# roxas1533/pathtrace

Measured on AMD Instinct MI355X. Metric: Msamples/sec (pixels x spp / s) at 1024^2/64spp, higher is better.
Workload: dtype f32; 1 GPU; C2: 10-sphere diffuse Cornell scene, 1024x1024, 64 spp, MIS, min_depth 4 / max_depth 50; hit_scene=linear scan (reference), launch=one process, one GPU, tiles=whole image

## Files before the change

include/pathtrace_amd.h:

```cpp
#ifndef PATHTRACE_AMD_H
#define PATHTRACE_AMD_H

#include <stdint.h>

#ifdef __cplusplus
extern "C" {
#endif

#define PT_ABI_VERSION 6

typedef enum {
    PT_OK = 0,
    PT_ERR_INVALID_ARG = 1,
    PT_ERR_NO_DEVICE = 2,
    PT_ERR_HIP = 3,
    PT_ERR_OOM = 4,
    PT_ERR_UNSUPPORTED = 5
} PtStatus;


typedef struct {
    double origin[3];
    double lower_left[3];
    double horizontal[3];
// ... 204 lines not shown
                                float* out_noisy_linear, float* out_features);

int pt_ray_color(PtContext* ctx, const PtRenderParams* params, const double* rays,
                 const uint32_t* xy, uint32_t n, float* out_rgb);

int pt_debug_hit_scene(PtContext* ctx, const double* rays, uint32_t n,
                       double t_min, double t_max, uint32_t exact_math, uint32_t accel,
                       int32_t* out_id, float* out_t);

int pt_debug_hit_records(PtContext* ctx, const double* rays, uint32_t n,
                         double t_min, double t_max, uint32_t exact_math, uint32_t accel,
                         int32_t* out_id, float* out_rec);

int pt_debug_bsdf_eval(PtContext* ctx, uint32_t obj, const double* in10, uint32_t n, uint32_t exact_math, float* out4);
int pt_debug_bsdf_sample(PtContext* ctx, uint32_t obj, const double* in7, const uint32_t* words4, uint32_t n,
                         uint32_t exact_math, float* out8);
int pt_debug_shape_sample(PtContext* ctx, uint32_t obj, const double* from3, const double* target3, const double* r12,
                          uint32_t n, uint32_t exact_math, float* out8);
int pt_debug_light_point(PtContext* ctx, const double* from3, const uint32_t* words4, uint32_t n, uint32_t exact_math,
                         float* out8);
int pt_debug_camera_rays(PtContext* ctx, const PtCamera* cam, const uint32_t* xys, uint32_t n, uint32_t exact_math,
                         float* out8);

int pt_debug_bvh_check(const PtObject* objs, uint32_t n_objs, uint32_t* depth, uint32_t* n_nodes,
                       uint32_t* n_leaf_slots);

const char* pt_last_error(void);
uint32_t pt_abi_version(void);

#ifdef __cplusplus
}
#endif
#endif
```

pathtrace_amd/_lib.py:

```python
import ctypes as C
import os

_HERE = os.path.dirname(os.path.abspath(__file__))
LIB_PATH = os.environ.get("PATHTRACE_AMD_LIB") or os.path.join(_HERE, "libpathtrace_amd.so")


class PtCamera(C.Structure):
    _fields_ = [
        ("origin", C.c_double * 3),
        ("lower_left", C.c_double * 3),
        ("horizontal", C.c_double * 3),
        ("vertical", C.c_double * 3),
        ("width", C.c_uint32),
        ("height", C.c_uint32),
    ]


class PtObject(C.Structure):
    _fields_ = [
        ("shape_tag", C.c_uint32),
        ("mat_tag", C.c_uint32),
        ("shape", C.c_double * 9),
        ("mat", C.c_double * 6),
    ]
# ... 120 lines not shown
    "pt_context_set_tuning": (C.c_int, [C.c_void_p, _P(PtTuning)]),
    "pt_scene_upload": (C.c_int, [C.c_void_p, _P(PtObject), C.c_uint32]),
    "pt_render_device": (C.c_int, [C.c_void_p, _P(PtCamera), _P(PtRenderParams), C.c_void_p, C.c_void_p]),
    "pt_render_device_packed": (C.c_int, [C.c_void_p, _P(PtCamera), _P(PtRenderParams), C.c_void_p]),
    "pt_sync": (C.c_int, [C.c_void_p]),
    "pt_get_stats": (C.c_int, [C.c_void_p, _P(PtStats)]),
    "pt_debug_raw_stats": (C.c_int, [C.c_void_p, _P(C.c_uint64)]),
    "pt_debug_scan_layout": (C.c_int, [C.c_void_p, _P(C.c_uint32), _P(C.c_uint32), _P(C.c_uint32)]),
    "pt_render_host": (C.c_int, [C.c_void_p, _P(PtCamera), _P(PtRenderParams), C.c_void_p, C.c_void_p]),
    "pt_render_progressive": (C.c_int, [C.c_void_p, _P(PtCamera), _P(PtRenderParams), C.c_uint32, C.c_void_p,
                                        C.c_void_p, C.c_void_p, C.c_void_p]),
    "pt_render": (C.c_int, [_P(PtCamera), _P(PtObject), C.c_uint32, _P(PtRenderParams), C.c_void_p, C.c_void_p]),
    "pt_debug_hit_scene": (C.c_int, [C.c_void_p, _P(C.c_double), C.c_uint32, C.c_double, C.c_double, C.c_uint32,
                                     C.c_uint32, _P(C.c_int32), _P(C.c_float)]),
    "pt_debug_hit_records": (C.c_int, [C.c_void_p, _P(C.c_double), C.c_uint32, C.c_double, C.c_double, C.c_uint32,
                                       C.c_uint32, _P(C.c_int32), _P(C.c_float)]),
    "pt_debug_bsdf_eval": (C.c_int, [C.c_void_p, C.c_uint32, _P(C.c_double), C.c_uint32, C.c_uint32, _P(C.c_float)]),
    "pt_debug_bsdf_sample": (C.c_int, [C.c_void_p, C.c_uint32, _P(C.c_double), _P(C.c_uint32), C.c_uint32, C.c_uint32,
                                       _P(C.c_float)]),
    "pt_debug_shape_sample": (C.c_int, [C.c_void_p, C.c_uint32, _P(C.c_double), _P(C.c_double), _P(C.c_double), C.c_uint32,
                                        C.c_uint32, _P(C.c_float)]),
    "pt_debug_light_point": (C.c_int, [C.c_void_p, _P(C.c_double), _P(C.c_uint32), C.c_uint32, C.c_uint32, _P(C.c_float)]),
    "pt_debug_camera_rays": (C.c_int, [C.c_void_p, _P(PtCamera), _P(C.c_uint32), C.c_uint32, C.c_uint32, _P(C.c_float)]),
    "pt_debug_bvh_check": (C.c_int, [_P(PtObject), C.c_uint32, _P(C.c_uint32), _P(C.c_uint32), _P(C.c_uint32)]),
    "pt_render_pixels": (C.c_int, [C.c_void_p, _P(PtCamera), _P(PtRenderParams), _P(C.c_uint32), C.c_uint32, C.c_void_p,
                                   C.c_void_p, C.c_void_p]),
    "pt_render_adaptive": (C.c_int, [C.c_void_p, _P(PtCamera), _P(PtRenderParams), _P(PtAdaptive), C.c_void_p, C.c_void_p,
                                     C.c_void_p, C.c_void_p]),
    "pt_render_features_device": (C.c_int, [C.c_void_p, _P(PtCamera), _P(PtRenderParams), C.c_uint32, C.c_void_p]),
    "pt_default_denoise": (None, [_P(PtDenoise)]),
    "pt_denoise_device": (C.c_int, [C.c_void_p, C.c_uint32, C.c_uint32, C.c_void_p, C.c_void_p, _P(PtDenoise), C.c_void_p, C.c_void_p]),
    "pt_render_denoised": (C.c_int, [C.c_void_p, _P(PtCamera), _P(PtRenderParams), C.c_uint32, _P(PtDenoise), C.c_void_p, C.c_void_p,
                                     C.c_void_p, C.c_void_p]),
    "pt_default_temporal": (None, [_P(PtTemporal)]),
    "pt_temporal_reset": (C.c_int, [C.c_void_p]),
    "pt_denoise_temporal_device": (C.c_int, [C.c_void_p, _P(PtCamera), C.c_void_p, C.c_void_p, _P(PtDenoise), _P(PtTemporal), C.c_void_p,
                                             C.c_void_p]),
    "pt_render_denoised_temporal": (C.c_int, [C.c_void_p, _P(PtCamera), _P(PtRenderParams), C.c_uint32, _P(PtDenoise), _P(PtTemporal),
                                              C.c_void_p, C.c_void_p, C.c_void_p, C.c_void_p]),
    "pt_ray_color": (C.c_int, [C.c_void_p, _P(PtRenderParams), _P(C.c_double), _P(C.c_uint32), C.c_uint32, C.c_void_p]),
    "pt_shutdown": (None, []),
    "pt_multi_create": (C.c_int, [_P(C.c_int), C.c_uint32, _P(C.c_void_p)]),
    "pt_multi_destroy": (C.c_int, [C.c_void_p]),
    "pt_multi_device_count": (C.c_uint32, [C.c_void_p]),
    "pt_multi_set_threads": (C.c_int, [C.c_void_p, C.c_int]),
    "pt_multi_set_exchange": (C.c_int, [C.c_void_p, C.c_uint32]),
# ... 60 lines not shown
```

pathtrace_amd/csrc/pt_api.cpp:

```cpp
#include <algorithm>
#include <cmath>
#include <cstdarg>
#include <cstdio>
#include <cstdlib>
#include <cstring>
#include <mutex>
#include <string>
#include <vector>

#include "../../include/pathtrace_amd.h"
#include "pt_bvh.h"
#include "pt_kernels.h"
#include "pt_sched.h"

#ifdef PT_SAN_NO_KERNELS
namespace ptk {
uint32_t launch_path_kernel_exact(const BounceArgs&, uint32_t, hipStream_t) { std::abort(); }
uint32_t launch_path_kernel_fast(const BounceArgs&, uint32_t, hipStream_t) { std::abort(); }
void launch_resolve_adaptive(const AdaptiveResolveArgs&, hipStream_t) { std::abort(); }
void launch_adaptive_select(const uint2*, uint32_t, uint32_t, const uint32_t*, uint32_t*, uint2*, uint32_t*, hipStream_t) { std::abort(); }
void launch_feature_rays_exact(const CameraF&, uint32_t, uint32_t, float*, hipStream_t) { std::abort(); }
void launch_feature_rays_fast(const CameraF&, uint32_t, uint32_t, float*, hipStream_t) { std::abort(); }
void launch_feature_resolve_exact(const FeatureResolveArgs&, hipStream_t) { std::abort(); }
void launch_feature_resolve_fast(const FeatureResolveArgs&, hipStream_t) { std::abort(); }
// ... 1166 lines not shown
                          uint32_t n, uint32_t exact_math, float* out8) {
    if ((!from3 || (!target3 && !r12)) && n) return fail(PT_ERR_INVALID_ARG, "null argument");
    std::vector<float> in(9 * (size_t)n, 0.0f);
    for (size_t i = 0; i < n; ++i) {
        for (int k = 0; k < 3; ++k) in[9 * i + k] = (float)from3[3 * i + k];
        if (target3) { for (int k = 0; k < 3; ++k) in[9 * i + 3 + k] = (float)target3[3 * i + k]; in[9 * i + 8] = 1.0f; }
        else { in[9 * i + 6] = (float)r12[2 * i]; in[9 * i + 7] = (float)r12[2 * i + 1]; }
    }
    return debug_fn(c, ptk::kFnShapeSample, obj, in, 9, nullptr, n, 8, exact_math, nullptr, out8);
}
int pt_debug_light_point(PtContext* c, const double* from3, const uint32_t* words4, uint32_t n, uint32_t exact_math,
                         float* out8) {
    if ((!from3 || !words4) && n) return fail(PT_ERR_INVALID_ARG, "null argument");
    return debug_fn(c, ptk::kFnLightPoint, 0, to_f32(from3, 3 * (size_t)n), 3, words4, n, 8, exact_math, nullptr, out8);
}
int pt_debug_camera_rays(PtContext* c, const PtCamera* cam, const uint32_t* xys, uint32_t n, uint32_t exact_math, float* out8) {
    if ((!cam || !xys) && n) return fail(PT_ERR_INVALID_ARG, "null argument");
    if (cam && (cam->width < 2 || cam->height < 2)) return fail(PT_ERR_INVALID_ARG, "camera %ux%u: width and height must be >= 2", cam->width, cam->height);
    std::vector<uint32_t> w(4 * (size_t)n, 0u);
    for (size_t i = 0; i < n; ++i) { w[4 * i] = xys[3 * i]; w[4 * i + 1] = xys[3 * i + 1]; w[4 * i + 2] = xys[3 * i + 2]; }
    return debug_fn(c, ptk::kFnCameraRay, 0, std::vector<float>(), 1, w.data(), n, 8, exact_math, cam, out8);
}

int pt_debug_bvh_check(const PtObject* objs, uint32_t n, uint32_t* depth, uint32_t* n_nodes, uint32_t* n_leaf_slots) {
    if (!objs && n) return fail(PT_ERR_INVALID_ARG, "pt_debug_bvh_check: null objects");
    if (n >= (1u << 28)) return fail(PT_ERR_UNSUPPORTED, "accel: %u objects exceed the 2^28 leaf slots", n);
    std::vector<float4> shape(3 * (size_t)n + 1), scan(3 * (size_t)n + 1);
    std::vector<uint32_t> tag(n + 1);
    for (uint32_t i = 0; i < n; ++i) {
        if (objs[i].shape_tag > PT_SHAPE_TRIANGLE) return fail(PT_ERR_INVALID_ARG, "object %u: bad shape_tag %u", i, objs[i].shape_tag);
        int ns = 0;
        shape_records(objs[i], &shape[3 * (size_t)i], &scan[3 * (size_t)i], &ns);
        tag[i] = objs[i].shape_tag;
    }
    const ptbvh::Built b = ptbvh::build(shape.data(), tag.data(), n);
    if (depth) *depth = b.depth;
    if (n_nodes) *n_nodes = (uint32_t)b.wide.size();
    if (n_leaf_slots) *n_leaf_slots = b.leaf_prims;
    if (b.non_finite) return fail(PT_ERR_UNSUPPORTED, "accel: %u object(s) with a NaN/inf coordinate", b.non_finite);
    if (b.depth + 2u > ptbvh::kStackDepth || b.stack_need > ptbvh::kStackDepth)
        return fail(PT_ERR_UNSUPPORTED, "BVH (depth %u, stack need %u) exceeds the traversal stack", b.depth, b.stack_need);
    if (b.leaf_prims != n || b.leaf_rec.size() != 3 * b.leaf_ids.size() || b.leaf_lead.size() != b.leaf_ids.size() || b.leaf_ids.size() % 4u != 0u)
        return fail(PT_ERR_UNSUPPORTED, "%u primitives in %zu leaf slots for %u objects", b.leaf_prims, b.leaf_ids.size(), n);
    if (n == 0) return b.root == ptbvh::kDone ? PT_OK : fail(PT_ERR_UNSUPPORTED, "empty scene: root is not the sentinel");
    auto prim_box = [&](uint32_t o, double lo[3], double hi[3]) {
        const float4 r0 = shape[3 * (size_t)o], r1 = shape[3 * (size_t)o + 1], r2 = shape[3 * (size_t)o + 2];
// ... 521 lines not shown
```

pathtrace_amd/csrc/pt_kernels.h:

```cpp
#pragma once
#include <hip/hip_runtime.h>
#include <stdint.h>

namespace ptk {

enum { kRunSphere = 0, kRunTriangle = 1, kRunTrianglePair = 2 };
struct Run {
    uint32_t tag;
    uint32_t first_obj;
    uint32_t count;
    uint32_t off4;
};
constexpr uint32_t run_entry_f4(uint32_t tag) { return tag == kRunSphere ? 1u : tag == kRunTriangle ? 3u : 5u; }

struct BvhView {
    const uint4* nodes;
    float grid_min[3], grid_cell[3];
    const float4* rec;
    const float4* lead;
    const uint32_t* ids;
    uint32_t root;
    float scene_abs;
};

// ... 139 lines not shown
    AdaptiveFilm f;
    const Rgb* lsamp;
    const uint2* pixels;
    uint32_t width, n, nb, n_total;
    uint32_t load;
    uint32_t finalize;
    uint32_t* zero_words;
    uint32_t n_zero;
};
void launch_resolve_adaptive(const AdaptiveResolveArgs& a, hipStream_t st);
constexpr uint32_t kSelectTile = 1024;
void launch_adaptive_select(const uint2* pixels, uint32_t n, uint32_t width, const uint32_t* conv, uint32_t* block_counts,
                            uint2* out, uint32_t* out_n, hipStream_t st);

void launch_film_pack(const float* lin, const uint8_t* rgba, uint32_t np, void* packed, hipStream_t st);
void launch_film_unpack(const void* recv, uint32_t W, uint32_t H, uint32_t band_rows, uint32_t n_dev, uint32_t max_rows, float* lin,
                        uint8_t* rgba, hipStream_t st);

void launch_debug_hit_exact(const SceneView& sc, uint32_t accel, const float* rays6, uint32_t n, float t_min, float t_max,
                            float4* scratch, int32_t* out_id, float* out_t, float* out_rec, hipStream_t st);
void launch_debug_hit_fast(const SceneView& sc, uint32_t accel, const float* rays6, uint32_t n, float t_min, float t_max,
                           float4* scratch, int32_t* out_id, float* out_t, float* out_rec, hipStream_t st);

enum { kFnBsdfEval = 0, kFnBsdfSample = 1, kFnShapeSample = 2, kFnLightPoint = 3, kFnCameraRay = 4 };
struct DebugFnArgs {
    SceneView sc;
    CameraF cam;
    uint32_t op, obj, n;
    uint32_t in_stride, out_stride;
    const float* in;
    const uint32_t* words;
    float* out;
};
void launch_debug_fn_exact(const DebugFnArgs& a, hipStream_t st);
void launch_debug_fn_fast(const DebugFnArgs& a, hipStream_t st);


struct FeatureResolveArgs {
    const float4* mat;
    const int32_t* ids;
    const float* rec;
    float4* out;
    uint32_t np, nb, n_samples, load, finalize;
};
void launch_feature_rays_exact(const CameraF& cam, uint32_t s_base, uint32_t nb, float* rays6, hipStream_t st);
void launch_feature_rays_fast(const CameraF& cam, uint32_t s_base, uint32_t nb, float* rays6, hipStream_t st);
void launch_feature_resolve_exact(const FeatureResolveArgs& a, hipStream_t st);
// ... 26 lines not shown
```

pathtrace_amd/csrc/pt_kernels.hip:

```cpp
#include "pt_device.h"
#include "pt_kernels.h"
#include "pt_adaptive.h"

using namespace PTD_NS;
using namespace ptk;

#if PT_MATH_EXACT
#define PTK_IMPL ptk_exact_impl
#define PT_LAUNCH(name) name##_exact
#else
#define PTK_IMPL ptk_fast_impl
#define PT_LAUNCH(name) name##_fast
#endif

#ifndef PT_TU
#define PT_TU 0
#endif
#define PT_TU_MAIN (PT_TU == 0 || PT_TU == 1)
#define PT_TU_SPLIT (PT_TU == 0 || PT_TU == 2)
#define PT_TU_BVH (PT_TU == 0 || PT_TU == 3)
namespace PTK_IMPL {

template <bool ORDERED = false, bool ANY = false>
PT_DEV void sphere_test(float4 s, f3 o, f3 d, float t_min, float& closest, int& id, int obj) {
// ... 190 lines not shown
    for (uint32_t r = 0; r < sc.n_runs; ++r) {
        Run run = sc.runs[r];
        run.tag = __builtin_amdgcn_readfirstlane(run.tag); run.first_obj = __builtin_amdgcn_readfirstlane(run.first_obj);
        run.count = __builtin_amdgcn_readfirstlane(run.count); run.off4 = __builtin_amdgcn_readfirstlane(run.off4);
        const uint32_t per = run_entry_f4(run.tag);
        if (SMALL) {
            scan_run<false, ANY, PF>(sc.scan + run.off4, run.tag, run.count, (int)run.first_obj, o, d, t_min, closest, id);
        } else {
            float4* tile = const_cast<float4*>(sc.scan);
            const uint32_t tile_prims = kTileF4 / per;
            for (uint32_t p0 = 0; p0 < run.count; p0 += tile_prims) {
                uint32_t np = run.count - p0 < tile_prims ? run.count - p0 : tile_prims;
                __syncthreads();
                const float4* src = sc.scan_global + run.off4 + p0 * per;
                for (uint32_t k = threadIdx.x; k < np * per; k += kBlock) tile[k] = src[k];
                __syncthreads();
                scan_run<true, ANY>(tile, run.tag, np, (int)(run.first_obj + p0 * (run.tag == kRunTrianglePair ? 2u : 1u)), o, d, t_min, closest, id);
            }
        }
    }
    id_out = id;
    t_out = closest;
}
PT_DEV void scan_global(const SceneRef& sc, f3 o, f3 d, float t_min, float t_max, int& id_out, float& t_out) {
    float closest = t_max;
    int id = -1;
    for (uint32_t r = 0; r < sc.n_runs; ++r) {
        const Run run = sc.runs_global[r];
        scan_run<false>(sc.scan_global + run.off4, run.tag, run.count, (int)run.first_obj, o, d, t_min, closest, id);
    }
    id_out = id;
    t_out = closest;
}

PT_DEV f3 parked_origin() { return mk(3e18f, 3e18f, 3e18f); }
PT_DEV f3 parked_dir() { return mk(1.0f, 0.0f, 0.0f); }

PT_DEV uint32_t lane_rank(unsigned long long mask) {
    return __builtin_amdgcn_mbcnt_hi((uint32_t)(mask >> 32), __builtin_amdgcn_mbcnt_lo((uint32_t)mask, 0u));
}
PT_DEV void divmod_magic(uint32_t n, uint32_t d, uint32_t magic, uint32_t& q, uint32_t& r) {
    q = __umulhi(n, magic);
    r = n - q * d;
    if (r >= d) { q += 1u; r -= d; }
}
PT_DEV uint32_t image_row(const TileMap& t, uint32_t yl) {
// ... 136 lines not shown
    v.light_dir = mk(0.f, 0.f, 0.f); v.ls_emission = mk(0.f, 0.f, 0.f);
    v.distance = 0.0f; v.ls_pdf = 1.0f;
    v.w_bsdf1 = v.w_bsdf2 = v.w_lobe = v.w_rr = 0u;
    if (v.alive) {
        uint32_t ds[4];
        philox4x32_draw(kx, py, sample, p.depth, BLK_SURFACE, 0u, ds);
        v.w_bsdf1 = ds[2]; v.w_bsdf2 = ds[3];
        v.w_rr = (ds[0] << 23) | ((ds[1] & 0x1FFu) << 14) | ((ds[2] & 0x1FFu) << 5);
        if (MIS && sc.n_lights > 0u) {
            uint32_t w_index = 0u;
            if (sc.n_lights > 1u) {
                uint32_t dc[4];
                philox4x32_draw(kx, py, sample, p.depth, BLK_CHOICE, 0u, dc);
                w_index = dc[0]; v.w_lobe = dc[1];
            }
            f3 lp;
            sample_light_point<DIFFUSE>(sc, v.hit.point, w_index, ds[0], ds[1], lp, v.light_obj, v.ls_emission, v.ls_pdf,
                                        v.light_dir, v.distance);
            v.need_shadow = true;
        }
    }
}

template <bool MIS, int DIFFUSE, bool REMAT>
PT_DEV bool vertex_end(const SceneRef& sc, PathState& p, const Vertex& vin, bool visible, uint32_t sample, uint32_t kx,
                       uint32_t py, uint32_t min_depth, uint32_t max_depth) {
    const uint32_t n_lights = sc.n_lights;
    Vertex v = vin;
    if (REMAT) {
        asm volatile("" ::: "memory");
        v.m = load_mat(sc.mat, vin.obj);
        v.ls_emission = load_mat(sc.mat, vin.light_obj).color;
    }
    if (DIFFUSE != kMatsMirror) assume_mats<DIFFUSE>(v.m.tag);
    else if (vin.alive) assume_mats<DIFFUSE>(v.m.tag);
    if (vin.hit_emitter) {
        if (!MIS || p.depth == 0u) {
            p.L = p.L + p.beta * v.m.color;
        } else {
            float w_bsdf = pt_div(p.pdf_prev, p.pdf_prev + vin.emit_pdf_shape);
            p.L = p.L + p.beta * v.m.color * w_bsdf;
        }
    }
    f3 direct = mk(0.f, 0.f, 0.f);
    if (MIS && visible) {
        float cos_theta = __builtin_fabsf(dot(v.hit.normal, v.light_dir));
        f3 bsdf; float pdf_bsdf;
        bsdf_pdf(v.m, p.d, p.eta_in, v.light_dir, v.hit.normal, bsdf, pdf_bsdf);
        float w_nee = pt_div(v.ls_pdf, v.ls_pdf + pdf_bsdf);
        direct = w_nee * bsdf * v.ls_emission * cos_theta / v.ls_pdf;
    }

    bool alive = v.alive;
    if (alive) {
        uint32_t w_lobe = v.w_lobe, w_rr = v.w_rr;
        if (!(MIS && n_lights > 1u) && v.m.tag == MAT_MIRROR) {
            uint32_t dc[4];
            philox4x32_draw(kx, py, sample, p.depth, BLK_CHOICE, 0u, dc);
            w_lobe = dc[1];
        }
        float eta_mat = v.m.tag == MAT_MIRROR ? v.m.ior : 1.0f;
        float eta_here = v.hit.front_face ? pt_rcp(eta_mat) : eta_mat;
        f3 wo, bsdf; float pdf, cos_theta;
        bsdf_pdf_sample(v.m, p.d, eta_here, v.hit.normal, v.w_bsdf1, v.w_bsdf2, w_lobe, wo, bsdf, pdf, cos_theta);
        f3 next_tp = p.beta * bsdf * cos_theta / pdf;
        float rr = rr_prob(p.depth, min_depth, max_depth, next_tp);
        if (u01(w_rr) > rr) {
            alive = false;
        } else {
            p.L = p.L + p.beta * direct;
            p.beta = rr == 1.0f ? next_tp : next_tp / rr;
            if (is_zero(p.beta) || p.depth >= 65534u) {
                alive = false;
            } else {
                p.pdf_prev = pdf;
                p.o = v.hit.point;
                p.d = v.m.tag == MAT_EMISSIVE ? normalize(wo) : wo;
                p.eta_in = eta_here;
                p.depth += 1u;
            }
        }
    }
    return alive;
}

#ifndef PT_BOUNCE_WAVES_LDS
#define PT_BOUNCE_WAVES_LDS 6
#endif
#ifndef PT_BOUNCE_WAVES_TILED
#define PT_BOUNCE_WAVES_TILED 5
#endif
template <bool LIST>
PT_DEV void pixel_key(const BounceArgs& a, const PathState& p, bool active, uint32_t& kx, uint32_t& py) {
    if (LIST) { const uint2 k = a.pixels[active ? ((p.yl << 16) | p.px) : 0u]; kx = k.x; py = k.y; }
    else { kx = p.px; py = image_row(a.tile, p.yl); }
}
// ... 144 lines not shown
        const uint32_t base = s_iters[0];
        if (threadIdx.x < n_in) {
#pragma unroll 1
            for (int k = 0; k < 4; ++k) { const float4 t = a.q.q[k][seg_base + threadIdx.x]; a.ovf_out.q[k][base + threadIdx.x] = t; }
        }
    }
    if (lane == 0u) wave_totals<MIS, !OVF>(s_totals, kBlock / 64, a.stats, wave_shadow, wave_vertices, wave_samples, wave_depth);
}

constexpr uint32_t kPool = 128;
#ifndef PT_REGEN_BLOCK
#define PT_REGEN_BLOCK 256
#endif
constexpr uint32_t kRegenBlock = PT_REGEN_BLOCK;
#ifndef PT_RESOLVE_UNROLL
#define PT_RESOLVE_UNROLL 4
#endif
template <bool MIS, int DIFFUSE, bool LIST = false>
__global__ void __launch_bounds__(kRegenBlock, DIFFUSE == kMatsDiffuse ? kRegenWavesDiffuse : kRegenWavesGeneric) k_paths_regen(BounceArgs a) {
    extern __shared__ float4 lds[];
    __shared__ float4 s_pool_d[kRegenBlock / 64][kPool];
    __shared__ uint32_t s_pool_s[kRegenBlock / 64][kPool];
    __shared__ WgTotals s_totals;
    if (threadIdx.x == 0u) wg_totals_init(s_totals);
    if (a.posted != nullptr && blockIdx.x >= a.core_blocks) {
        __shared__ uint32_t s_posted;
        if (threadIdx.x == 0u) s_posted = __hip_atomic_load(a.posted, __ATOMIC_RELAXED, __HIP_MEMORY_SCOPE_SYSTEM);
        __syncthreads();
        if (s_posted - a.seq >= 2u) return;
    }
    const SceneRef sc = stage_scene<kModeLds>(a.sc, lds);
    const uint32_t lane = threadIdx.x & 63u;
    const uint32_t wib = threadIdx.x >> 6;
    float4* const pool_d = s_pool_d[wib];
    uint32_t* const pool_s = s_pool_s[wib];
    const uint32_t n_first = a.n_first;
    const uint32_t n_chunks = (n_first + 63u) >> 6;
    const uint32_t W = a.film_w;
    const f3 cam_o = mk(a.cam.origin[0], a.cam.origin[1], a.cam.origin[2]);

    const uint32_t wave = blockIdx.x * (kRegenBlock / 64) + wib, nw = gridDim.x * (kRegenBlock / 64);
    uint32_t st_next = wave;
    uint32_t ctr = blockIdx.x % kRegenCounters, ctr_dry = 0;
    uint32_t pool_head = 0, pool_cnt = 0;
    bool exhausted = false;
    uint32_t wave_shadow = 0, wave_vertices = 0;
    uint32_t wave_taken = 0;
    uint32_t dmax = 0;
    PathState p = parked_state();
    bool alive = false;
#ifdef PT_DRAIN_TIMING
    const unsigned long long t_begin = wall_clock64();
    unsigned long long t_exhausted = 0ull;
#endif

    for (;;) {
#ifdef PT_DRAIN_TIMING
        if (exhausted && t_exhausted == 0ull) t_exhausted = wall_clock64();
#endif
        while (!exhausted && pool_cnt < 64u) {
            uint32_t chunk;
            if (st_next < a.regen_static) {
                chunk = st_next; st_next += nw;
            } else {
                for (;;) {
                    uint32_t got = 0;
                    if (lane == 0u) got = atomicAdd(a.chunk_counter + ctr * kRegenCounterStride, 1u);
                    chunk = a.regen_static + __builtin_amdgcn_readfirstlane(got) * kRegenCounters + ctr;
                    if (chunk < n_chunks) break;
                    ctr = ctr + 1u == kRegenCounters ? 0u : ctr + 1u;
                    if (++ctr_dry == kRegenCounters) { exhausted = true; break; }
                }
                if (exhausted) break;
            }
            const uint32_t pid = chunk * 64u + lane;
            const uint32_t valid = n_first - chunk * 64u < 64u ? n_first - chunk * 64u : 64u;
            if (lane < valid) {
                uint32_t s_local, pix, yl, px;
                divmod_magic(pid, a.np, a.np_magic, s_local, pix);
                divmod_magic(pix, W, a.film_w_magic, yl, px);
                f3 o, d;
                if constexpr (LIST) { const uint2 k = a.pixels[pix]; camera_ray(a.cam, a.s_base + s_local, k.x, k.y, o, d); }
                else camera_ray(a.cam, a.s_base + s_local, px, image_row(a.tile, yl), o, d);
                const uint32_t e = (pool_head + pool_cnt + lane) & (kPool - 1u);
                pool_d[e] = make_float4(d.x, d.y, d.z, __uint_as_float((yl << 16) | px));
                pool_s[e] = s_local << 16;
            }
            pool_cnt += valid;
        }
        __builtin_amdgcn_wave_barrier();
        {
            const unsigned long long need = __ballot(!alive);
            const uint32_t r = lane_rank(need);
            if (!alive && r < pool_cnt) {
                const uint32_t e = (pool_head + r) & (kPool - 1u);
                const float4 q = pool_d[e];
                const uint32_t sd = pool_s[e];
                p.o = cam_o; p.d = mk(q.x, q.y, q.z);
                const uint32_t xy = __float_as_uint(q.w);
                p.yl = xy >> 16; p.px = xy & 0xFFFFu;
                p.s_local = sd >> 16; p.depth = 0u;
                p.beta = mk(1.f, 1.f, 1.f); p.L = mk(0.f, 0.f, 0.f);
                p.pdf_prev = 0.0f; p.eta_in = 1.0f;
                alive = true;
            }
            const uint32_t n_need = (uint32_t)__popcll(need);
            const uint32_t n_take = n_need < pool_cnt ? n_need : pool_cnt;
            pool_head += n_take; pool_cnt -= n_take;
            wave_taken += n_take;
        }
        __builtin_amdgcn_wave_barrier();
        const uint32_t n_alive = (uint32_t)__popcll(__ballot(alive));
        if (n_alive < a.export_below) break;

        const bool active = alive;
        uint32_t kx = p.px, py = image_row(a.tile, p.yl);
        if constexpr (LIST) pixel_key<true>(a, p, active, kx, py);
        const uint32_t sample = a.s_base + p.s_local;
        wave_vertices += n_alive;

        int id; float t;
        scan_closest<kModeLds, false>(sc, p.o, p.d, a.t_min, kInf, id, t);
        Vertex v;
        vertex_begin<MIS, DIFFUSE>(sc, p, active, id, t, sample, kx, py, v);

        bool visible = false;
        if (MIS) {
            const unsigned long long sm = __ballot(v.need_shadow);
            if (sm != 0ull) {
                f3 sdir = v.need_shadow ? v.light_dir : parked_dir();
                f3 sorg = v.need_shadow ? v.hit.point : parked_origin();
                int sid; float st;
                scan_closest<kModeLds, true>(sc, sorg, sdir, a.t_min, v.distance - a.t_min, sid, st);
                visible = v.need_shadow && sid < 0;
                wave_shadow += (uint32_t)__popcll(sm);
            }
        }
        alive = vertex_end<MIS, DIFFUSE, true>(sc, p, v, visible, sample, kx, py, a.min_depth, a.max_depth);
        if (active && !alive) {
            a.lsamp[p.s_local * a.np + p.yl * W + p.px] = Rgb{p.L.x, p.L.y, p.L.z};
            dmax = p.depth > dmax ? p.depth : dmax;
            p.o = parked_origin(); p.d = parked_dir();
        }
    }

    {
        const unsigned long long mask = __ballot(alive);
        const uint32_t n_left = (uint32_t)__popcll(mask);
        if (n_left != 0u) {
            uint32_t base = 0;
            if (lane == 0u) base = atomicAdd(a.ovf_out_count, n_left);
            base = __builtin_amdgcn_readfirstlane(base);
            if (alive) {
                store_state(a.ovf_out, base + lane_rank(mask), p);
                const uint32_t done = p.depth ? p.depth - 1u : 0u;
                dmax = done > dmax ? done : dmax;
            }
        }
        wave_taken -= n_left;
    }
    const uint32_t wave_samples = wave_taken;
    for (int off = 32; off > 0; off >>= 1) { const uint32_t w2 = (uint32_t)__shfl_xor((int)dmax, off); dmax = w2 > dmax ? w2 : dmax; }
    if (lane == 0u) {
        wave_totals<MIS>(s_totals, kRegenBlock / 64, a.stats, wave_shadow, wave_vertices, wave_samples, dmax);
#ifdef PT_DRAIN_TIMING
// ... 915 lines not shown
        const bool with_target = in[8] != 0.0f;
        shape_sample(sc.shape, sc.mat, (int)a.obj, m.shape_tag, from, with_target, mk(in[3], in[4], in[5]), in[6], in[7], point, pdf, dir, dist);
        if (with_target) {
            const f3 to_light = point - from;
            dir = normalize(to_light); dist = length(to_light);
        }
        out[0] = point.x; out[1] = point.y; out[2] = point.z; out[3] = pdf;
        out[4] = dir.x; out[5] = dir.y; out[6] = dir.z; out[7] = dist;
    } else if (a.op == kFnLightPoint) {
        f3 point = mk(0.f, 0.f, 0.f), le = point, ld = point; float pdf = 0.0f, ll = 0.0f; int lobj = -1;
        if (sc.n_lights > 0u) sample_light_point<false>(sc, mk(in[0], in[1], in[2]), w[0], w[1], w[2], point, lobj, le, pdf, ld, ll);
        out[0] = point.x; out[1] = point.y; out[2] = point.z; out[3] = le.x; out[4] = le.y; out[5] = le.z;
        out[6] = pdf; out[7] = (float)lobj;
    } else if (a.op == kFnCameraRay) {
        f3 o, d;
        camera_ray(a.cam, w[2], w[0], w[1], o, d);
        uint32_t dc[4];
        philox4x32_draw(w[0], w[1], w[2], kDepthCamera, BLK_SURFACE, 0u, dc);
        out[0] = o.x; out[1] = o.y; out[2] = o.z; out[3] = d.x; out[4] = d.y; out[5] = d.z;
        out[6] = u01(dc[0]); out[7] = u01(dc[1]);
    }
}

__global__ void k_scene_setup(float4* shape, float4* mat, uint32_t n) {
    const uint32_t i = blockIdx.x * blockDim.x + threadIdx.x;
    if (i >= n) return;
    const uint32_t bits = __float_as_uint(mat[2 * i].x);
    if (((bits >> 8) & 0xFFu) != SHAPE_TRIANGLE) return;
    float4 r0 = shape[3 * i], r1 = shape[3 * i + 1], r2 = shape[3 * i + 2];
    f3 normal; float pdf_area;
    triangle_constants(mk(r1.x, r1.y, r1.z), mk(r2.x, r2.y, r2.z), normal, pdf_area);
    r0.w = normal.x; r1.w = normal.y; r2.w = normal.z;
    shape[3 * i] = r0; shape[3 * i + 1] = r1; shape[3 * i + 2] = r2;
    mat[2 * i + 1].w = pdf_area;
}
#endif
}
namespace ptk {
using namespace PTK_IMPL;
#if PT_TU_BVH
void PT_LAUNCH(launch_debug_hit_bvh)(const SceneView& sc, uint32_t grid, size_t lds, const float* rays6, uint32_t n, float t_min, float t_max,
                                     float4* scratch, int32_t* out_id, float* out_t, float* out_rec, hipStream_t st) {
    hipLaunchKernelGGL(k_debug_hit_bvh, dim3(grid), dim3(kBlock), lds, st, sc, rays6, n, t_min, t_max, scratch,
                       scratch + n, scratch + 2 * (size_t)n, out_id, out_t, out_rec);
}
#endif
#if PT_TU_MAIN
void PT_LAUNCH(launch_scene_setup)(float4* shape, float4* mat, uint32_t n, hipStream_t st) {
    if (n == 0u) return;
    hipLaunchKernelGGL(k_scene_setup, dim3((n + kBlock - 1) / kBlock), dim3(kBlock), 0, st, shape, mat, n);
}
void PT_LAUNCH(launch_debug_fn)(const DebugFnArgs& a, hipStream_t st) {
    if (a.n == 0u) return;
    hipLaunchKernelGGL(k_debug_fn, dim3((a.n + kBlock - 1) / kBlock), dim3(kBlock), 0, st, a);
}
void PT_LAUNCH(launch_debug_hit)(const SceneView& sc, uint32_t accel, const float* rays6, uint32_t n, float t_min,
                                 float t_max, float4* scratch, int32_t* out_id, float* out_t, float* out_rec, hipStream_t st) {
    const int mode = scene_mode(sc, accel);
    const size_t lds = scene_lds_bytes(sc, mode);
    uint32_t grid = (n + kBlock - 1) / kBlock;
    if (grid > 2048u) grid = 2048u;
    if (grid == 0u) grid = 1u;
    if (mode == kModeLds)
        hipLaunchKernelGGL(k_debug_hit<kModeLds>, dim3(grid), dim3(kBlock), lds, st, sc, rays6, n, t_min, t_max, out_id, out_t, out_rec);
    else if (mode == kModeTiled)
        hipLaunchKernelGGL(k_debug_hit<kModeTiled>, dim3(grid), dim3(kBlock), lds, st, sc, rays6, n, t_min, t_max, out_id, out_t, out_rec);
    else
        PT_LAUNCH(launch_debug_hit_bvh)(sc, grid, lds, rays6, n, t_min, t_max, scratch, out_id, out_t, out_rec, st);
}
#endif

}

#if PT_TU_MAIN
namespace PTK_IMPL {
__global__ void __launch_bounds__(kBlock) k_feature_rays(CameraF cam, uint32_t s_base, uint32_t nb, float* __restrict__ rays6) {
// ... 269 lines not shown
```

rust/pathtrace-amd-sys/src/lib.rs:

```rust
#![allow(non_camel_case_types)]
use std::os::raw::{c_char, c_int, c_void};

pub const PT_ABI_VERSION: u32 = 6;

pub const PT_OK: c_int = 0;
pub const PT_ERR_INVALID_ARG: c_int = 1;
pub const PT_ERR_NO_DEVICE: c_int = 2;
pub const PT_ERR_HIP: c_int = 3;
pub const PT_ERR_OOM: c_int = 4;
pub const PT_ERR_UNSUPPORTED: c_int = 5;

pub const PT_SHAPE_SPHERE: u32 = 0;
pub const PT_SHAPE_TRIANGLE: u32 = 1;
pub const PT_MAT_LAMBERT: u32 = 0;
pub const PT_MAT_EMISSIVE: u32 = 1;
pub const PT_MAT_MIRROR: u32 = 2;
pub const PT_MAT_OREN_NAYAR: u32 = 3;
pub const PT_INTEGRATOR_MIS: u32 = 0;
pub const PT_INTEGRATOR_BRDF_ONLY: u32 = 1;
pub const PT_ACCEL_LINEAR: u32 = 0;
pub const PT_ACCEL_BVH: u32 = 1;
pub const PT_ACCEL_AUTO: u32 = 2;

#[repr(C)]
// ... 213 lines not shown
    pub fn pt_multi_render_host(m: *mut PtMulti, cam: *const PtCamera, params: *const PtRenderParams, out_linear_rgb: *mut f32, out_rgba8: *mut u8) -> c_int;
    pub fn pt_render_multi(devices: *const c_int, n_devices: u32, cam: *const PtCamera, objs: *const PtObject, n_objs: u32, params: *const PtRenderParams, out_linear_rgb: *mut f32, out_rgba8: *mut u8) -> c_int;
    pub fn pt_film_pack(hip_stream: *mut c_void, d_linear_rgb: *const f32, d_rgba8: *const u8, n_pixels: u32, d_packed: *mut c_void) -> c_int;
    pub fn pt_film_unpack(hip_stream: *mut c_void, d_gathered: *const c_void, width: u32, height: u32, band_rows: u32, n_ranks: u32, max_rows: u32, d_linear_rgb: *mut f32, d_rgba8: *mut u8) -> c_int;
    pub fn pt_debug_multi_emulate(ctx: *mut PtContext, n_virtual: u32, cam: *const PtCamera, params: *const PtRenderParams, out_linear_rgb: *mut f32, out_rgba8: *mut u8) -> c_int;
    pub fn pt_render_pixels(ctx: *mut PtContext, cam: *const PtCamera, params: *const PtRenderParams, xy: *const u32, n: u32, out_linear_rgb: *mut f32, out_rgba8: *mut u8, out_samples: *mut f32) -> c_int;
    pub fn pt_render_adaptive(ctx: *mut PtContext, cam: *const PtCamera, params: *const PtRenderParams, ad: *const PtAdaptive, out_linear_rgb: *mut f32, out_rgba8: *mut u8, out_spp: *mut u32, out_rel_err: *mut f32) -> c_int;
    pub fn pt_render_features_device(ctx: *mut PtContext, cam: *const PtCamera, params: *const PtRenderParams, n_samples: u32, d_features: *mut f32) -> c_int;
    pub fn pt_default_denoise(out: *mut PtDenoise);
    pub fn pt_denoise_device(ctx: *mut PtContext, width: u32, height: u32, d_linear_rgb: *const f32, d_features: *const f32, dn: *const PtDenoise, d_out_linear: *mut f32, d_out_rgba8: *mut u8) -> c_int;
    pub fn pt_render_denoised(ctx: *mut PtContext, cam: *const PtCamera, params: *const PtRenderParams, feature_samples: u32, dn: *const PtDenoise, out_linear_rgb: *mut f32, out_rgba8: *mut u8, out_noisy_linear: *mut f32, out_features: *mut f32) -> c_int;
    pub fn pt_default_temporal(out: *mut PtTemporal);
    pub fn pt_temporal_reset(ctx: *mut PtContext) -> c_int;
    pub fn pt_denoise_temporal_device(ctx: *mut PtContext, cam: *const PtCamera, d_linear_rgb: *const f32, d_features: *const f32, dn: *const PtDenoise, tp: *const PtTemporal, d_out_linear: *mut f32, d_out_rgba8: *mut u8) -> c_int;
    pub fn pt_render_denoised_temporal(ctx: *mut PtContext, cam: *const PtCamera, params: *const PtRenderParams, feature_samples: u32, dn: *const PtDenoise, tp: *const PtTemporal, out_linear_rgb: *mut f32, out_rgba8: *mut u8, out_noisy_linear: *mut f32, out_features: *mut f32) -> c_int;
    pub fn pt_ray_color(ctx: *mut PtContext, params: *const PtRenderParams, rays: *const f64, xy: *const u32, n: u32, out_rgb: *mut f32) -> c_int;
    pub fn pt_debug_hit_scene(ctx: *mut PtContext, rays: *const f64, n: u32, t_min: f64, t_max: f64, exact_math: u32, accel: u32, out_id: *mut i32, out_t: *mut f32) -> c_int;
    pub fn pt_debug_hit_records(ctx: *mut PtContext, rays: *const f64, n: u32, t_min: f64, t_max: f64, exact_math: u32, accel: u32, out_id: *mut i32, out_rec: *mut f32) -> c_int;
    pub fn pt_debug_bsdf_eval(ctx: *mut PtContext, obj: u32, in10: *const f64, n: u32, exact_math: u32, out4: *mut f32) -> c_int;
    pub fn pt_debug_bsdf_sample(ctx: *mut PtContext, obj: u32, in7: *const f64, words4: *const u32, n: u32, exact_math: u32, out8: *mut f32) -> c_int;
    pub fn pt_debug_shape_sample(ctx: *mut PtContext, obj: u32, from3: *const f64, target3: *const f64, r12: *const f64, n: u32, exact_math: u32, out8: *mut f32) -> c_int;
    pub fn pt_debug_light_point(ctx: *mut PtContext, from3: *const f64, words4: *const u32, n: u32, exact_math: u32, out8: *mut f32) -> c_int;
    pub fn pt_debug_camera_rays(ctx: *mut PtContext, cam: *const PtCamera, xys: *const u32, n: u32, exact_math: u32, out8: *mut f32) -> c_int;
    pub fn pt_debug_bvh_check(objs: *const PtObject, n_objs: u32, depth: *mut u32, n_nodes: *mut u32, n_leaf_slots: *mut u32) -> c_int;
    pub fn pt_last_error() -> *const c_char;
    pub fn pt_abi_version() -> u32;
}
```

Before: 12470 Msamples/s.

## Defer MIS shadow test and fuse it with next bounce's closest-hit scan

```diff
diff --git a/include/pathtrace_amd.h b/include/pathtrace_amd.h
--- a/include/pathtrace_amd.h
+++ b/include/pathtrace_amd.h
@@ -250,6 +250,9 @@
 int pt_debug_camera_rays(PtContext* ctx, const PtCamera* cam, const uint32_t* xys, uint32_t n, uint32_t exact_math,
                          float* out8);
 
+int pt_debug_joint_scan(PtContext* ctx, const double* rays10, uint32_t n, double t_min, double t_max_b,
+                        uint32_t exact_math, float* out6);
+
 int pt_debug_bvh_check(const PtObject* objs, uint32_t n_objs, uint32_t* depth, uint32_t* n_nodes,
                        uint32_t* n_leaf_slots);
 
diff --git a/pathtrace_amd/_lib.py b/pathtrace_amd/_lib.py
--- a/pathtrace_amd/_lib.py
+++ b/pathtrace_amd/_lib.py
@@ -166,6 +166,7 @@
                                         C.c_uint32, _P(C.c_float)]),
     "pt_debug_light_point": (C.c_int, [C.c_void_p, _P(C.c_double), _P(C.c_uint32), C.c_uint32, C.c_uint32, _P(C.c_float)]),
     "pt_debug_camera_rays": (C.c_int, [C.c_void_p, _P(PtCamera), _P(C.c_uint32), C.c_uint32, C.c_uint32, _P(C.c_float)]),
+    "pt_debug_joint_scan": (C.c_int, [C.c_void_p, _P(C.c_double), C.c_uint32, C.c_double, C.c_double, C.c_uint32, _P(C.c_float)]),
     "pt_debug_bvh_check": (C.c_int, [_P(PtObject), C.c_uint32, _P(C.c_uint32), _P(C.c_uint32), _P(C.c_uint32)]),
     "pt_render_pixels": (C.c_int, [C.c_void_p, _P(PtCamera), _P(PtRenderParams), _P(C.c_uint32), C.c_uint32, C.c_void_p,
                                    C.c_void_p, C.c_void_p]),
diff --git a/pathtrace_amd/csrc/pt_api.cpp b/pathtrace_amd/csrc/pt_api.cpp
--- a/pathtrace_amd/csrc/pt_api.cpp
+++ b/pathtrace_amd/csrc/pt_api.cpp
@@ -1212,6 +1212,18 @@
     return debug_fn(c, ptk::kFnCameraRay, 0, std::vector<float>(), 1, w.data(), n, 8, exact_math, cam, out8);
 }
 
+int pt_debug_joint_scan(PtContext* c, const double* rays10, uint32_t n, double t_min, double t_max_b, uint32_t exact_math, float* out6) {
+    if (!rays10 && n) return fail(PT_ERR_INVALID_ARG, "null argument");
+    if (c && c->has_scene && (c->view.n_objs > ptk::kSmallObjs || c->view.blob_f4 == 0))
+        return fail(PT_ERR_UNSUPPORTED, "pt_debug_joint_scan: the scene (%u objects) does not live in LDS", c->view.n_objs);
+    std::vector<float> in(12 * (size_t)n);
+    for (size_t i = 0; i < n; ++i) {
+        for (int k = 0; k < 10; ++k) in[12 * i + k] = (float)rays10[10 * i + k];
+        in[12 * i + 10] = (float)t_min; in[12 * i + 11] = (float)t_max_b;
+    }
+    return debug_fn(c, ptk::kFnJointScan, 0, in, 12, nullptr, n, 6, exact_math, nullptr, out6);
+}
+
 int pt_debug_bvh_check(const PtObject* objs, uint32_t n, uint32_t* depth, uint32_t* n_nodes, uint32_t* n_leaf_slots) {
     if (!objs && n) return fail(PT_ERR_INVALID_ARG, "pt_debug_bvh_check: null objects");
     if (n >= (1u << 28)) return fail(PT_ERR_UNSUPPORTED, "accel: %u objects exceed the 2^28 leaf slots", n);
diff --git a/pathtrace_amd/csrc/pt_kernels.h b/pathtrace_amd/csrc/pt_kernels.h
--- a/pathtrace_amd/csrc/pt_kernels.h
+++ b/pathtrace_amd/csrc/pt_kernels.h
@@ -185,7 +185,8 @@
 void launch_debug_hit_fast(const SceneView& sc, uint32_t accel, const float* rays6, uint32_t n, float t_min, float t_max,
                            float4* scratch, int32_t* out_id, float* out_t, float* out_rec, hipStream_t st);
 
-enum { kFnBsdfEval = 0, kFnBsdfSample = 1, kFnShapeSample = 2, kFnLightPoint = 3, kFnCameraRay = 4 };
+enum { kFnBsdfEval = 0, kFnBsdfSample = 1, kFnShapeSample = 2, kFnLightPoint = 3, kFnCameraRay = 4,
+       kFnJointScan = 5 };
 struct DebugFnArgs {
     SceneView sc;
     CameraF cam;
diff --git a/pathtrace_amd/csrc/pt_kernels.hip b/pathtrace_amd/csrc/pt_kernels.hip
--- a/pathtrace_amd/csrc/pt_kernels.hip
+++ b/pathtrace_amd/csrc/pt_kernels.hip
@@ -236,6 +236,76 @@
     id_out = id;
     t_out = closest;
 }
+PT_DEV void sphere_pre2(float4 s, f3 o, f3 da, f3 db, float& half_a, float& disc_a, float& half_b, float& disc_b) {
+    const f3 oc = o - mk(s.x, s.y, s.z);
+    half_a = dot(oc, da);
+    half_b = dot(oc, db);
+    const f3 la = madd(da, -half_a, oc);
+    const f3 lb = madd(db, -half_b, oc);
+    disc_a = s.w - dot(la, la);
+    disc_b = s.w - dot(lb, lb);
+}
+PT_DEV void sphere_post2(float ha, float da, float hb, float db, float t_min, float bound_a, int& id_a, float& closest, int& id, int obj) {
+    sphere_post<true>(ha, da, t_min, bound_a, id_a, obj);
+    sphere_post<false>(hb, db, t_min, closest, id, obj);
+}
+PT_DEV void scan_run2(const float4* __restrict__ p, uint32_t tag, uint32_t n, int first_obj, f3 o, f3 da, f3 db, float t_min,
+                      float bound_a, int& id_a, float& closest, int& id) {
+    if (tag == SHAPE_SPHERE) {
+        uint32_t i = 0;
+        for (; i + 4u <= n; i += 4u) {
+            const float4 s0 = p[i], s1 = p[i + 1], s2 = p[i + 2], s3 = p[i + 3];
+            float ha0, ha1, ha2, ha3, da0, da1, da2, da3, hb0, hb1, hb2, hb3, db0, db1, db2, db3;
+            sphere_pre2(s0, o, da, db, ha0, da0, hb0, db0); sphere_pre2(s1, o, da, db, ha1, da1, hb1, db1);
+            sphere_pre2(s2, o, da, db, ha2, da2, hb2, db2); sphere_pre2(s3, o, da, db, ha3, da3, hb3, db3);
+            sphere_post2(ha0, da0, hb0, db0, t_min, bound_a, id_a, closest, id, first_obj + (int)i);
+            sphere_post2(ha1, da1, hb1, db1, t_min, bound_a, id_a, closest, id, first_obj + (int)i + 1);
+            sphere_post2(ha2, da2, hb2, db2, t_min, bound_a, id_a, closest, id, first_obj + (int)i + 2);
+            sphere_post2(ha3, da3, hb3, db3, t_min, bound_a, id_a, closest, id, first_obj + (int)i + 3);
+        }
+        if (i + 2u <= n) {
+            const float4 s0 = p[i], s1 = p[i + 1];
+            float ha0, ha1, da0, da1, hb0, hb1, db0, db1;
+            sphere_pre2(s0, o, da, db, ha0, da0, hb0, db0); sphere_pre2(s1, o, da, db, ha1, da1, hb1, db1);
+            sphere_post2(ha0, da0, hb0, db0, t_min, bound_a, id_a, closest, id, first_obj + (int)i);
+            sphere_post2(ha1, da1, hb1, db1, t_min, bound_a, id_a, closest, id, first_obj + (int)i + 1);
+            i += 2u;
+        }
+        for (; i < n; ++i) {
+            float ha0, da0, hb0, db0;
+            sphere_pre2(p[i], o, da, db, ha0, da0, hb0, db0);
+            sphere_post2(ha0, da0, hb0, db0, t_min, bound_a, id_a, closest, id, first_obj + (int)i);
+        }
+    } else if (tag == kRunTriangle) {
+        for (uint32_t i = 0; i < n; ++i) {
+            const float4 a0 = p[3 * i], a1 = p[3 * i + 1], a2 = p[3 * i + 2];
+            float ca = bound_a;
+            triangle_test<false, true>(a0, a1, a2, o, da, t_min, ca, id_a, first_obj + (int)i);
+            triangle_test<false, false>(a0, a1, a2, o, db, t_min, closest, id, first_obj + (int)i);
+        }
+    } else {
+        for (uint32_t i = 0; i < n; ++i) {
+            const float4 a0 = p[5 * i], a1 = p[5 * i + 1], a2 = p[5 * i + 2], a3 = p[5 * i + 3], a4 = p[5 * i + 4];
+            float ca = bound_a;
+            tripair_test<true>(a0, a1, a2, a3, a4, o, da, t_min, ca, id_a, first_obj + 2 * (int)i);
+            tripair_test<false>(a0, a1, a2, a3, a4, o, db, t_min, closest, id, first_obj + 2 * (int)i);
+        }
+    }
+}
+template <int MODE>
+PT_DEV void scan_closest2(const SceneRef& sc, f3 o, f3 da, float t_max_a, f3 db, float t_min, float t_max_b, int& id_a, int& id_b,
+                          float& t_b) {
+    static_assert(MODE == kModeLds, "the whole scan array in LDS");
+    float closest = t_max_b;
+    int ia = -1, ib = -1;
+    for (uint32_t r = 0; r < sc.n_runs; ++r) {
+        Run run = sc.runs[r];
+        run.tag = __builtin_amdgcn_readfirstlane(run.tag); run.first_obj = __builtin_amdgcn_readfirstlane(run.first_obj);
+        run.count = __builtin_amdgcn_readfirstlane(run.count); run.off4 = __builtin_amdgcn_readfirstlane(run.off4);
+        scan_run2(sc.scan + run.off4, run.tag, run.count, (int)run.first_obj, o, da, db, t_min, t_max_a, ia, closest, ib);
+    }
+    id_a = ia; id_b = ib; t_b = closest;
+}
 PT_DEV void scan_global(const SceneRef& sc, f3 o, f3 d, float t_min, float t_max, int& id_out, float& t_out) {
     float closest = t_max;
     int id = -1;
@@ -418,9 +488,20 @@
     }
 }
 
-template <bool MIS, int DIFFUSE, bool REMAT>
+struct Pending {
+    bool on;
+    f3 beta, direct;
+};
+PT_DEV void vertex_finish(PathState& p, Pending& pd, bool visible) {
+    if (pd.on) {
+        const f3 direct = visible ? pd.direct : mk(0.f, 0.f, 0.f);
+        p.L = p.L + pd.beta * direct;
+        pd.on = false;
+    }
+}
+template <bool MIS, int DIFFUSE, bool REMAT, bool DEFER = false>
 PT_DEV bool vertex_end(const SceneRef& sc, PathState& p, const Vertex& vin, bool visible, uint32_t sample, uint32_t kx,
-                       uint32_t py, uint32_t min_depth, uint32_t max_depth) {
+                       uint32_t py, uint32_t min_depth, uint32_t max_depth, Pending* pd = nullptr) {
     const uint32_t n_lights = sc.n_lights;
     Vertex v = vin;
     if (REMAT) {
@@ -439,7 +520,7 @@
         }
     }
     f3 direct = mk(0.f, 0.f, 0.f);
-    if (MIS && visible) {
+    if (MIS && (DEFER ? vin.need_shadow : visible)) {
         float cos_theta = __builtin_fabsf(dot(v.hit.normal, v.light_dir));
         f3 bsdf; float pdf_bsdf;
         bsdf_pdf(v.m, p.d, p.eta_in, v.light_dir, v.hit.normal, bsdf, pdf_bsdf);
@@ -464,10 +545,12 @@
         if (u01(w_rr) > rr) {
             alive = false;
         } else {
-            p.L = p.L + p.beta * direct;
+            if (DEFER) { pd->on = true; pd->beta = p.beta; pd->direct = direct; }
+            else p.L = p.L + p.beta * direct;
             p.beta = rr == 1.0f ? next_tp : next_tp / rr;
             if (is_zero(p.beta) || p.depth >= 65534u) {
                 alive = false;
+                if (DEFER) p.o = v.hit.point;
             } else {
                 p.pdf_prev = pdf;
                 p.o = v.hit.point;
@@ -658,6 +741,7 @@
     __shared__ float4 s_pool_d[kRegenBlock / 64][kPool];
     __shared__ uint32_t s_pool_s[kRegenBlock / 64][kPool];
     __shared__ WgTotals s_totals;
+    __shared__ float4 s_park[MIS ? kRegenBlock / 64 : 1][2][64];
     if (threadIdx.x == 0u) wg_totals_init(s_totals);
     if (a.posted != nullptr && blockIdx.x >= a.core_blocks) {
         __shared__ uint32_t s_posted;
@@ -670,6 +754,8 @@
     const uint32_t wib = threadIdx.x >> 6;
     float4* const pool_d = s_pool_d[wib];
     uint32_t* const pool_s = s_pool_s[wib];
+    float4* const park0 = &s_park[MIS ? wib : 0u][0][lane];
+    float4* const park1 = &s_park[MIS ? wib : 0u][1][lane];
     const uint32_t n_first = a.n_first;
     const uint32_t n_chunks = (n_first + 63u) >> 6;
     const uint32_t W = a.film_w;
@@ -685,6 +771,24 @@
     uint32_t dmax = 0;
     PathState p = parked_state();
     bool alive = false;
+    Pending pd;
+    pd.on = false; pd.beta = mk(0.f, 0.f, 0.f); pd.direct = mk(0.f, 0.f, 0.f);
+    f3 sdir = parked_dir();
+    float smax = -1.0f;
+    auto park = [&]() {
+        *park0 = make_float4(pd.beta.x, pd.beta.y, pd.beta.z, pd.direct.x);
+        *park1 = make_float4(pd.direct.y, pd.direct.z, 0.0f, 0.0f);
+    };
+    auto unpark = [&]() {
+        asm volatile("" ::: "memory");
+        const float4 k0 = *park0, k1 = *park1;
+        pd.beta = mk(k0.x, k0.y, k0.z); pd.direct = mk(k0.w, k1.x, k1.y);
+    };
+    auto retire = [&]() {
+        a.lsamp[p.s_local * a.np + p.yl * W + p.px] = Rgb{p.L.x, p.L.y, p.L.z};
+        dmax = p.depth > dmax ? p.depth : dmax;
+        p.o = parked_origin(); p.d = parked_dir();
+    };
 #ifdef PT_DRAIN_TIMING
     const unsigned long long t_begin = wall_clock64();
     unsigned long long t_exhausted = 0ull;
@@ -726,9 +830,10 @@
         }
         __builtin_amdgcn_wave_barrier();
         {
-            const unsigned long long need = __ballot(!alive);
+            const bool vacant = !alive && !(MIS && pd.on);
+            const unsigned long long need = __ballot(vacant);
             const uint32_t r = lane_rank(need);
-            if (!alive && r < pool_cnt) {
+            if (vacant && r < pool_cnt) {
                 const uint32_t e = (pool_head + r) & (kPool - 1u);
                 const float4 q = pool_d[e];
                 const uint32_t sd = pool_s[e];
@@ -747,7 +852,8 @@
         }
         __builtin_amdgcn_wave_barrier();
         const uint32_t n_alive = (uint32_t)__popcll(__ballot(alive));
-        if (n_alive < a.export_below) break;
+        const uint32_t n_busy = MIS ? (uint32_t)__popcll(__ballot(alive || pd.on)) : n_alive;
+        if (n_busy < a.export_below) break;
 
         const bool active = alive;
         uint32_t kx = p.px, py = image_row(a.tile, p.yl);
@@ -755,28 +861,44 @@
         const uint32_t sample = a.s_base + p.s_local;
         wave_vertices += n_alive;
 
-        int id; float t;
-        scan_closest<kModeLds, false>(sc, p.o, p.d, a.t_min, kInf, id, t);
-        Vertex v;
-        vertex_begin<MIS, DIFFUSE>(sc, p, active, id, t, sample, kx, py, v);
-
-        bool visible = false;
-        if (MIS) {
-            const unsigned long long sm = __ballot(v.need_shadow);
-            if (sm != 0ull) {
-                f3 sdir = v.need_shadow ? v.light_dir : parked_dir();
-                f3 sorg = v.need_shadow ? v.hit.point : parked_origin();
-                int sid; float st;
-                scan_closest<kModeLds, true>(sc, sorg, sdir, a.t_min, v.distance - a.t_min, sid, st);
-                visible = v.need_shadow && sid < 0;
-                wave_shadow += (uint32_t)__popcll(sm);
-            }
-        }
-        alive = vertex_end<MIS, DIFFUSE, true>(sc, p, v, visible, sample, kx, py, a.min_depth, a.max_depth);
-        if (active && !alive) {
-            a.lsamp[p.s_local * a.np + p.yl * W + p.px] = Rgb{p.L.x, p.L.y, p.L.z};
-            dmax = p.depth > dmax ? p.depth : dmax;
-            p.o = parked_origin(); p.d = parked_dir();
+        if constexpr (MIS) {
+            const bool shadow = pd.on && sc.n_lights > 0u;
+            int id, sid = -1; float t;
+            if (__ballot(shadow) != 0ull)
+                scan_closest2<kModeLds>(sc, p.o, shadow ? sdir : p.d, shadow ? smax : -1.0f, p.d, a.t_min, kInf, sid, id, t);
+            else
+                scan_closest<kModeLds, false>(sc, p.o, p.d, a.t_min, kInf, id, t);
+            const bool ended = pd.on && !alive;
+            unpark();
+            vertex_finish(p, pd, shadow && sid < 0);
+            if (ended) retire();
+            Vertex v;
+            vertex_begin<MIS, DIFFUSE>(sc, p, active, id, t, sample, kx, py, v);
+            wave_shadow += (uint32_t)__popcll(__ballot(v.need_shadow));
+            alive = vertex_end<MIS, DIFFUSE, true, true>(sc, p, v, false, sample, kx, py, a.min_depth, a.max_depth, &pd);
+            sdir = v.light_dir; smax = v.distance - a.t_min;
+            park();
+            if (active && !alive && !pd.on) retire();
+        } else {
+            int id; float t;
+            scan_closest<kModeLds, false>(sc, p.o, p.d, a.t_min, kInf, id, t);
+            Vertex v;
+            vertex_begin<MIS, DIFFUSE>(sc, p, active, id, t, sample, kx, py, v);
+            alive = vertex_end<MIS, DIFFUSE, true>(sc, p, v, false, sample, kx, py, a.min_depth, a.max_depth);
+            if (active && !alive) retire();
+        }
+    }
+
+    if constexpr (MIS) {
+        if (__ballot(pd.on) != 0ull) {
+            const bool shadow = pd.on && sc.n_lights > 0u;
+            int sid = -1; float st;
+            if (__ballot(shadow) != 0ull)
+                scan_closest<kModeLds, true>(sc, shadow ? p.o : parked_origin(), shadow ? sdir : parked_dir(), a.t_min, smax, sid, st);
+            const bool ended = pd.on && !alive;
+            unpark();
+            vertex_finish(p, pd, shadow && sid < 0);
+            if (ended) retire();
         }
     }
 
@@ -1738,6 +1860,30 @@
     }
 }
 
+__global__ void __launch_bounds__(kBlock) k_debug_scan2(DebugFnArgs a) {
+    extern __shared__ float4 lds[];
+    const SceneRef sc = stage_scene<kModeLds>(a.sc, lds);
+    const uint32_t i = blockIdx.x * kBlock + threadIdx.x;
+    const bool active = i < a.n;
+    f3 o = parked_origin(), da = parked_dir(), db = parked_dir();
+    float t_max_a = -1.0f, t_min = 0.0f, t_max_b = kInf;
+    if (active) {
+        const float* in = a.in + (size_t)i * a.in_stride;
+        o = mk(in[0], in[1], in[2]); da = mk(in[3], in[4], in[5]); db = mk(in[6], in[7], in[8]);
+        t_max_a = in[9]; t_min = in[10]; t_max_b = in[11];
+    }
+    int ja, jb, sa, sb; float jt, st, unused;
+    scan_closest2<kModeLds>(sc, o, da, t_max_a, db, t_min, t_max_b, ja, jb, jt);
+    asm volatile("" ::: "memory");
+    scan_closest<kModeLds, true>(sc, o, da, t_min, t_max_a, sa, unused);
+    scan_closest<kModeLds, false>(sc, o, db, t_min, t_max_b, sb, st);
+    if (active) {
+        float* out = a.out + (size_t)i * a.out_stride;
+        out[0] = __int_as_float(ja >= 0 ? 1 : 0); out[1] = __int_as_float(jb); out[2] = jt;
+        out[3] = __int_as_float(sa >= 0 ? 1 : 0); out[4] = __int_as_float(sb); out[5] = st;
+    }
+}
+
 __global__ void k_scene_setup(float4* shape, float4* mat, uint32_t n) {
     const uint32_t i = blockIdx.x * blockDim.x + threadIdx.x;
     if (i >= n) return;
@@ -1768,6 +1914,10 @@
 }
 void PT_LAUNCH(launch_debug_fn)(const DebugFnArgs& a, hipStream_t st) {
     if (a.n == 0u) return;
+    if (a.op == kFnJointScan) {
+        hipLaunchKernelGGL(k_debug_scan2, dim3((a.n + kBlock - 1) / kBlock), dim3(kBlock), scene_lds_bytes(a.sc, kModeLds), st, a);
+        return;
+    }
     hipLaunchKernelGGL(k_debug_fn, dim3((a.n + kBlock - 1) / kBlock), dim3(kBlock), 0, st, a);
 }
 void PT_LAUNCH(launch_debug_hit)(const SceneView& sc, uint32_t accel, const float* rays6, uint32_t n, float t_min,
diff --git a/rust/pathtrace-amd-sys/src/lib.rs b/rust/pathtrace-amd-sys/src/lib.rs
--- a/rust/pathtrace-amd-sys/src/lib.rs
+++ b/rust/pathtrace-amd-sys/src/lib.rs
@@ -259,6 +259,7 @@
     pub fn pt_debug_shape_sample(ctx: *mut PtContext, obj: u32, from3: *const f64, target3: *const f64, r12: *const f64, n: u32, exact_math: u32, out8: *mut f32) -> c_int;
     pub fn pt_debug_light_point(ctx: *mut PtContext, from3: *const f64, words4: *const u32, n: u32, exact_math: u32, out8: *mut f32) -> c_int;
     pub fn pt_debug_camera_rays(ctx: *mut PtContext, cam: *const PtCamera, xys: *const u32, n: u32, exact_math: u32, out8: *mut f32) -> c_int;
+    pub fn pt_debug_joint_scan(ctx: *mut PtContext, rays10: *const f64, n: u32, t_min: f64, t_max_b: f64, exact_math: u32, out6: *mut f32) -> c_int;
     pub fn pt_debug_bvh_check(objs: *const PtObject, n_objs: u32, depth: *mut u32, n_nodes: *mut u32, n_leaf_slots: *mut u32) -> c_int;
     pub fn pt_last_error() -> *const c_char;
     pub fn pt_abi_version() -> u32;
```

Measured after the change: 12880 Msamples/s, median of 6. +3.3%, better.
